# theEricMa/TriplaneTurbo

Hardware: AMD Instinct MI355X
Metric: rendered rays/sec (fwd+bwd) at 256x256 rays x 128 samples (higher is better)
Workload: dtype f32 (fp32-grade: exact 3-piece fp16 operand split, 6 x v_mfma_f32_32x32x16_f16 per k-step, fp32 accumulation)

## Files before the change

### triplaneturbo_amd/csrc/tt_backward_common.h

```cpp
#pragma once
#include "tt_device.h"
#include "tt_mfma16.h"
#include "tt_alpha.h"
#include "tt_launch.h"
#include <type_traits>

typedef int i32x4 __attribute__((ext_vector_type(4)));

#ifdef TT_TUNING
#define TT_PHASE(k)                                              \
    do {                                                         \
        __builtin_amdgcn_sched_barrier(0);                       \
        const unsigned long long t_now = __builtin_amdgcn_s_memtime(); \
        ph_acc[k] += t_now - ph_t;                               \
        ph_t = t_now;                                            \
        __builtin_amdgcn_sched_barrier(0);                       \
    } while (0)
#else
#define TT_PHASE(k) \
    do {            \
    } while (0)
#endif
#define XS 36

template <int N>
__device__ __forceinline__ void stage_rows(float* S, const float (&v)[N / 2], int j, int hi) {
#pragma unroll
    for (int r = 0; r < N / 2; ++r) S[LIDX(r, hi) * XS + j] = v[r];
}
template <int N, int OFF, int TOT>
__device__ __forceinline__ void stage_rows_sub(float* S, const float (&v)[TOT], int j, int hi) {
#pragma unroll
    for (int r = 0; r < N / 2; ++r) S[LIDX(r, hi) * XS + j] = v[OFF + r];
}
template <int N>
__device__ __forceinline__ void stage_rows_mask(float* S, const float (&v)[N / 2], int j, int hi) {
#pragma unroll
    for (int r = 0; r < N / 2; ++r) S[LIDX(r, hi) * XS + j] = v[r] > 0.f ? 1.f : 0.f;
}

template <int NX, int NY>
__device__ __forceinline__ void wgrad(f32x16 (&acc)[NX / 32][NY / 32], const float* Xs, const float* Ys, int i,
                                      int hi) {
#pragma unroll
    for (int t4 = 0; t4 < 4; ++t4) {
        f32x4 xa[NX / 32], yb[NY / 32];
#pragma unroll
        for (int m = 0; m < NX / 32; ++m)
            xa[m] = *reinterpret_cast<const f32x4*>(Xs + (32 * m + i) * XS + 16 * hi + 4 * t4);
#pragma unroll
        for (int n = 0; n < NY / 32; ++n)
            yb[n] = *reinterpret_cast<const f32x4*>(Ys + (32 * n + i) * XS + 16 * hi + 4 * t4);
#pragma unroll
        for (int k = 0; k < 4; ++k)
#pragma unroll
            for (int m = 0; m < NX / 32; ++m)
#pragma unroll
                for (int n = 0; n < NY / 32; ++n)
                    acc[m][n] = __builtin_amdgcn_mfma_f32_32x32x2f32(xa[m][k], yb[n][k], acc[m][n], 0, 0, 0);
    }
}

template <int NY>
__device__ __forceinline__ void wgrad_row(f32x16 (&acc)[NY / 32], const float* Xs, const float* Ys, int i, int hi) {
#pragma unroll
    for (int t4 = 0; t4 < 4; ++t4) {
        f32x4 yb[NY / 32];
        const f32x4 xa = *reinterpret_cast<const f32x4*>(Xs + i * XS + 16 * hi + 4 * t4);
#pragma unroll
        for (int n = 0; n < NY / 32; ++n)
            yb[n] = *reinterpret_cast<const f32x4*>(Ys + (32 * n + i) * XS + 16 * hi + 4 * t4);
#pragma unroll
        for (int k = 0; k < 4; ++k)
#pragma unroll
            for (int n = 0; n < NY / 32; ++n)
                acc[n] = __builtin_amdgcn_mfma_f32_32x32x2f32(xa[k], yb[n][k], acc[n], 0, 0, 0);
    }
}

typedef unsigned u32x4 __attribute__((ext_vector_type(4)));

__device__ __forceinline__ float wg16_scale(float bound) {
    int E = (int)(__builtin_bit_cast(unsigned, bound * 1.0001f) >> 23) & 0xff;
    E = E < 16 ? 16 : (E > 240 ? 240 : E);
    return __builtin_bit_cast(float, (unsigned)(268 - E) << 23);
}
__device__ __forceinline__ unsigned wg16_pack(float x) {
    unsigned out;
    float r;
    asm("v_cvt_pk_f16_f32 %0, %2, 0\n\t"
        "v_fma_mix_f32 %1, %2, 1.0, -%0 op_sel_hi:[0,0,1]\n\t"
        "v_cvt_pk_f16_f32 %0, %2, %1"
        : "=&v"(out), "=&v"(r)
        : "v"(x));
    return out;
}
template <int N>
__device__ __forceinline__ void stage_rows16(float* S, const float (&v)[N / 2], int j, int hi, float sc) {
    unsigned* U = reinterpret_cast<unsigned*>(S);
#pragma unroll
    for (int r = 0; r < N / 2; ++r) U[LIDX(r, hi) * XS + j] = wg16_pack(v[r] * sc);
}
template <int N, int OFF, int TOT>
__device__ __forceinline__ void stage_rows16_sub(float* S, const float (&v)[TOT], int j, int hi, float sc) {
    unsigned* U = reinterpret_cast<unsigned*>(S);
#pragma unroll
    for (int r = 0; r < N / 2; ++r) U[LIDX(r, hi) * XS + j] = wg16_pack(v[OFF + r] * sc);
}
template <int N, int PAIR, int NT>
__device__ __forceinline__ void stage_rows16_pre(float* S, const Split16<N, PAIR, NT>& v, int j, int hi) {
    unsigned* U = reinterpret_cast<unsigned*>(S);
#pragma unroll
    for (int t = 0; t < N / 4; ++t) {
        U[LIDX(pair_reg<PAIR>(t, 0), hi) * XS + j] = __builtin_amdgcn_perm(v.l[t], v.h[t], 0x05040100u);
        U[LIDX(pair_reg<PAIR>(t, 1), hi) * XS + j] = __builtin_amdgcn_perm(v.l[t], v.h[t], 0x07060302u);
    }
}
template <int N>
__device__ __forceinline__ void stage_rows16_mask(float* S, const unsigned (&mb)[N / 4], int j, int hi) {
    unsigned* U = reinterpret_cast<unsigned*>(S);
#pragma unroll
    for (int t = 0; t < N / 4; ++t) {
        U[LIDX(2 * t, hi) * XS + j] = __builtin_amdgcn_perm(0u, mb[t], 0x01000100u);
        U[LIDX(2 * t + 1, hi) * XS + j] = __builtin_amdgcn_perm(0u, mb[t], 0x03020302u);
    }
}
__device__ __forceinline__ h8_t wg16_frag(const float* S, int row, int t, int hi) {
    return __builtin_bit_cast(h8_t, *reinterpret_cast<const u32x4*>(S + row * XS + 8 * t + 4 * hi));
}
__device__ __forceinline__ h8_t wg16_swap(h8_t v) {
    u32x4 u = __builtin_bit_cast(u32x4, v);
#pragma unroll
    for (int d = 0; d < 4; ++d) u[d] = __builtin_amdgcn_alignbit(u[d], u[d], 16);
    return __builtin_bit_cast(h8_t, u);
}
template <int NX, int NY>
__device__ __forceinline__ void wgrad16(f32x16 (&acc)[NX / 32][NY / 32], const float* Xs, const float* Ys, int i,
                                        int hi) {
#pragma unroll
    for (int t = 0; t < 4; ++t) {
        h8_t xa[NX / 32], yb[NY / 32], ys[NY / 32];
#pragma unroll
        for (int m = 0; m < NX / 32; ++m) xa[m] = wg16_frag(Xs, 32 * m + i, t, hi);
#pragma unroll
        for (int n = 0; n < NY / 32; ++n) {
            yb[n] = wg16_frag(Ys, 32 * n + i, t, hi);
            ys[n] = wg16_swap(yb[n]);
        }
#pragma unroll
        for (int m = 0; m < NX / 32; ++m)
#pragma unroll
            for (int n = 0; n < NY / 32; ++n)
                acc[m][n] = __builtin_amdgcn_mfma_f32_32x32x16_f16(xa[m], yb[n], acc[m][n], 0, 0, 0);
#pragma unroll
        for (int m = 0; m < NX / 32; ++m)
#pragma unroll
            for (int n = 0; n < NY / 32; ++n)
                acc[m][n] = __builtin_amdgcn_mfma_f32_32x32x16_f16(xa[m], ys[n], acc[m][n], 0, 0, 0);
    }
}
template <int NX, int NY>
__device__ __forceinline__ void wgrad16_mask(f32x16 (&acc)[NX / 32][NY / 32], const float* Xs, const float* Ys, int i,
                                             int hi) {
#pragma unroll
    for (int t = 0; t < 4; ++t) {
        h8_t xa[NX / 32], yb[NY / 32];
#pragma unroll
        for (int m = 0; m < NX / 32; ++m) xa[m] = wg16_frag(Xs, 32 * m + i, t, hi);
#pragma unroll
        for (int n = 0; n < NY / 32; ++n) yb[n] = wg16_frag(Ys, 32 * n + i, t, hi);
#pragma unroll
        for (int m = 0; m < NX / 32; ++m)
#pragma unroll
            for (int n = 0; n < NY / 32; ++n)
                acc[m][n] = __builtin_amdgcn_mfma_f32_32x32x16_f16(xa[m], yb[n], acc[m][n], 0, 0, 0);
    }
}
template <int NY>
__device__ __forceinline__ void wgrad16_row(f32x16 (&acc)[NY / 32], const float* Xs, const float* Ys, int i, int hi) {
#pragma unroll
    for (int t = 0; t < 4; ++t) {
        const h8_t xa = wg16_frag(Xs, i, t, hi);
        h8_t yb[NY / 32], ys[NY / 32];
#pragma unroll
        for (int n = 0; n < NY / 32; ++n) {
            yb[n] = wg16_frag(Ys, 32 * n + i, t, hi);
            ys[n] = wg16_swap(yb[n]);
        }
#pragma unroll
        for (int n = 0; n < NY / 32; ++n) acc[n] = __builtin_amdgcn_mfma_f32_32x32x16_f16(xa, yb[n], acc[n], 0, 0, 0);
#pragma unroll
        for (int n = 0; n < NY / 32; ++n) acc[n] = __builtin_amdgcn_mfma_f32_32x32x16_f16(xa, ys[n], acc[n], 0, 0, 0);
    }
}

__device__ __forceinline__ float block_max(float v, unsigned* word) {
    __syncthreads();
    if (threadIdx.x == 0) *word = 0u;
    __syncthreads();
#pragma unroll
    for (int o = 32; o > 0; o >>= 1) v = fmaxf(v, __shfl_xor(v, o));
    if ((threadIdx.x & 63) == 0) atomicMax(word, __builtin_bit_cast(unsigned, v));
    __syncthreads();
    const float r = __builtin_bit_cast(float, *word);
    __syncthreads();
    return r;
}

template <class Addr>
__device__ __forceinline__ void flush_tile_reduced(float* R, int parity, const f32x16& acc, int wave, int lane,
                                                   float ux, float uy, Addr addr) {
    float* B = R + parity * 4096;
#pragma unroll
    for (int r = 0; r < 16; ++r) B[(wave * 16 + r) * 64 + lane] = (acc[r] * ux) * uy;
    __syncthreads();
#pragma unroll
    for (int q = 0; q < 4; ++q) {
        const int r = 4 * wave + q;
        const float v = (B[r * 64 + lane] + B[(16 + r) * 64 + lane]) + (B[(32 + r) * 64 + lane] + B[(48 + r) * 64 + lane]);
        atomicAdd(addr(r), v);
    }
}
template <int NX, int NY>
__device__ __forceinline__ void flush_wgrad_reduced(float* R, int& parity, const f32x16 (&acc)[NX / 32][NY / 32],
                                                    float* __restrict__ dst, int wave, int lane, float ux, float uy) {
    const int i = lane & 31, hi = lane >> 5;
#pragma unroll
    for (int m = 0; m < NX / 32; ++m)
#pragma unroll
        for (int n = 0; n < NY / 32; ++n) {
            flush_tile_reduced(R, parity, acc[m][n], wave, lane, ux, uy,
                               [&](int r) { return dst + (32 * m + LIDX(r, hi)) * NY + 32 * n + i; });
            parity ^= 1;
        }
}

template <int NX, int NY>
__device__ __forceinline__ void flush_d_reduced(float* R, int& parity, const f32x16 (&acc)[NX / 32][NY / 32],
                                                const float* __restrict__ W, const float* __restrict__ wo,
                                                float* __restrict__ dW, float* __restrict__ dwo, int wave, int lane,
                                                float uy) {
    const int i = lane & 31, hi = lane >> 5;
#pragma unroll
    for (int m = 0; m < NX / 32; ++m) {
        float part[4] = {0.f, 0.f, 0.f, 0.f};
#pragma unroll
        for (int n = 0; n < NY / 32; ++n) {
            float* B = R + parity * 4096;
#pragma unroll
            for (int r = 0; r < 16; ++r) B[(wave * 16 + r) * 64 + lane] = acc[m][n][r] * uy;
            __syncthreads();
#pragma unroll
            for (int q = 0; q < 4; ++q) {
                const int r = 4 * wave + q, at = (32 * m + LIDX(r, hi)) * NY + 32 * n + i;
                const float d = (B[r * 64 + lane] + B[(16 + r) * 64 + lane]) + (B[(32 + r) * 64 + lane] + B[(48 + r) * 64 + lane]);
                atomicAdd(dW + at, wo[32 * m + LIDX(r, hi)] * d);
                part[q] = fmaf(W[at], d, part[q]);
            }
            parity ^= 1;
        }
#pragma unroll
        for (int q = 0; q < 4; ++q) {
            float s = part[q];
#pragma unroll
            for (int o = 16; o > 0; o >>= 1) s += __shfl_xor(s, o);
            if (i == 0) atomicAdd(dwo + 32 * m + LIDX(4 * wave + q, hi), s);
        }
    }
}

#define ZERO16 \
    { 0.f, 0.f, 0.f, 0.f, 0.f, 0.f, 0.f, 0.f, 0.f, 0.f, 0.f, 0.f, 0.f, 0.f, 0.f, 0.f }

#define MS XS

#define M16_RS 40
#define M16_PLANE (65 * M16_RS)
#define SCATTER_M_FLOATS 2624
template <bool EXACT>
__device__ __forceinline__ void scatter_clear(float* M, int lane) {
    const f32x4 z = {0.f, 0.f, 0.f, 0.f};
    if (EXACT) {
#pragma unroll
        for (int g = 0; g < MS / 4; ++g) *reinterpret_cast<f32x4*>(M + lane * MS + 4 * g) = z;
    } else {
#pragma unroll
        for (int g = 0; g < SCATTER_M_FLOATS / 256; ++g) *reinterpret_cast<f32x4*>(M + (g * 64 + lane) * 4) = z;
        if (lane < (SCATTER_M_FLOATS % 256) / 4)
            *reinterpret_cast<f32x4*>(M + ((SCATTER_M_FLOATS / 256) * 64 + lane) * 4) = z;
    }
}

#define SCATTER_TAG_INTS 160
__device__ __forceinline__ float* sc2_factor_table(int* tags, int pl) { return reinterpret_cast<float*>(tags + 32) + 32 * pl; }

struct PlaneRefs {
    float c0, c1;
    int o0, o1;
    int h0, h1;
    float qs;
};
template <bool NORM>
__device__ __forceinline__ PlaneRefs plane_refs(const float (&coef)[4], const int (&aoff)[4], const int (&hs)[4],
                                                int hi) {
    PlaneRefs r;
    float cn = 1.f;
    r.qs = 1.f;
    if (NORM) {
        const float m = fmaxf(fmaxf(__builtin_fabsf(coef[0]), __builtin_fabsf(coef[1])),
                              fmaxf(__builtin_fabsf(coef[2]), __builtin_fabsf(coef[3])));
        int E = (int)(__builtin_bit_cast(unsigned, m) >> 23);
        E = E < 16 ? 16 : (E > 240 ? 240 : E);
        cn = __builtin_bit_cast(float, (unsigned)(268 - E) << 23);
        r.qs = __builtin_bit_cast(float, (unsigned)(E - 14) << 23);
    }
    r.c0 = (hi ? coef[2] : coef[0]) * cn;
    r.c1 = (hi ? coef[3] : coef[1]) * cn;
    r.o0 = hi ? aoff[2] : aoff[0];
    r.o1 = hi ? aoff[3] : aoff[1];
    r.h0 = hi ? hs[2] : hs[0];
    r.h1 = hi ? hs[3] : hs[1];
    return r;
}
__device__ __forceinline__ void scatter_init_tags(int* tags, int lane) {
    if (lane < 32) tags[lane] = -2;
}
// ... 518 lines not shown
```

### triplaneturbo_amd/csrc/tt_backward_tex.hip

```cpp
#include "tt_backward_common.h"

#define TEX_SCRATCH_FLOATS (128 * XS)
template <int PREC>
struct TexMap : LdsMap<PREC, LdsImage<64, 96>, LdsImage<64, 64>, LdsRows<3, 64>, LdsImage<96, 64, PREC != PREC_S3>,
                       LdsImage<64, 64, PREC != PREC_S3>> {
    static constexpr bool COPIES = PREC != PREC_S3;
    typedef typename TexMap::template at<0> V1;
    typedef typename TexMap::template at<1> V2;
    typedef typename TexMap::template at<2> V3;
    typedef typename TexMap::template at<3> V1T;
    typedef typename TexMap::template at<4> V2T;
};
__device__ __forceinline__ float uniform_f(float v) {
    return __builtin_bit_cast(float, __builtin_amdgcn_readfirstlane(__builtin_bit_cast(int, v)));
}

template <int PREC, bool WG16, bool STATS = false>
__global__ __launch_bounds__(256, 1) void k_decode_bwd_tex(BwdTexParams p) {
    constexpr bool EXACT = PREC == PREC_F32;
    typedef TexMap<PREC> F;
    constexpr int NT = PrecNT<PREC>::value, WF = F::FLOATS;
    __shared__ __attribute__((aligned(16))) float Lt[WF + 4 * (TEX_SCRATCH_FLOATS + SCATTER_TAG_INTS)];
    stage_weights<PREC>(Lt, typename F::V1{}, p.w.v1);
    stage_weights<PREC>(Lt, typename F::V2{}, p.w.v2);
    stage_weights<PREC>(Lt, typename F::V3{}, p.w.v3);
    if constexpr (F::COPIES) {
        stage_weights_t<PREC>(Lt, typename F::V1T{}, p.w.v1);
        stage_weights_t<PREC>(Lt, typename F::V2T{}, p.w.v2);
    }
    const tt_render_cfg& cfg = p.cfg;
    float sKB1 = 1.f, sE = 1.f, sK2B = 1.f, sK1 = 1.f;
    if (WG16) {
        const unsigned* bnd = reinterpret_cast<const unsigned*>(p.queue) + TT_SLOT_BOUNDS;
        const float Pm = __builtin_bit_cast(float, bnd[TT_BOUND_PLANES]), Gr = __builtin_bit_cast(float, bnd[TT_BOUND_UP0]),
                    Gf = __builtin_bit_cast(float, bnd[TT_BOUND_UP1]);
        unsigned* word = reinterpret_cast<unsigned*>(Lt + WF);
        const int t = threadIdx.x;
        const float CBmax = __builtin_fabsf(cfg.rgb_grad_shrink) * (1.002f * 0.25f) * Gr + Gf;
        float v1row = 0.f, k2b = 0.f, kb1 = 0.f;
        if (t < 64) {
            for (int c = 0; c < 96; ++c) v1row += __builtin_fabsf(p.w.v1[t * 96 + c]);
            for (int o = 0; o < 3; ++o) k2b += __builtin_fabsf(p.w.v3[o * 64 + t]);
            for (int r = 0; r < 64; ++r) {
                float c3 = 0.f;
                for (int o = 0; o < 3; ++o) c3 += __builtin_fabsf(p.w.v3[o * 64 + r]);
                kb1 += __builtin_fabsf(p.w.v2[r * 64 + t]) * c3;
            }
        }
        const float V1max = block_max(v1row, word), K2Bw = block_max(k2b, word), KB1w = block_max(kb1, word);
        sE = wg16_scale(Pm);
        sK1 = wg16_scale(V1max * Pm);
        sK2B = wg16_scale(K2Bw * CBmax);
        sKB1 = wg16_scale(KB1w * CBmax);
    }
    sE = uniform_f(sE), sK1 = uniform_f(sK1), sK2B = uniform_f(sK2B), sKB1 = uniform_f(sKB1);
    const float uE = uniform_f(1.f / sE), uK1 = uniform_f(1.f / sK1);
    const TileGeom& tg = p.geom;
    const int lane = threadIdx.x & 63, i = lane & 31, hi = lane >> 5,
              wave_in_blk = __builtin_amdgcn_readfirstlane((int)(threadIdx.x >> 6));
    float* Xs = Lt + WF + wave_in_blk * (TEX_SCRATCH_FLOATS + SCATTER_TAG_INTS);
    float* Ys = Xs + 32 * XS;
    int* tags = reinterpret_cast<int*>(Xs + 128 * XS);
    float* Cb = Xs + 32;
#define CB_AT(idx) Cb[((idx) >> 2) * XS + ((idx)&3)]
    scatter_init_tags(tags, lane);
    __syncthreads();
    const int S = cfg.n_samples;
    const int H = cfg.plane_h, W = cfg.plane_w;
    const size_t HW = (size_t)H * W;
    const size_t plane_stride = 6 * HW * TT_C;
    ItemQueue iq = item_queue(p.queue, tg.n_blocks, tg.n_chunks, tg.unit);
    const float shrink = cfg.rgb_grad_shrink;
    float* const grad_out =
        p.grad_packed + (size_t)(blockIdx.x % (unsigned)p.n_copies) * cfg.n_prompts * plane_stride;
    const unsigned grad_bytes =
        TT_DBG(cfg.flags, TT_DBG_NO_ATOMICS) ? 0u : (unsigned)(cfg.n_prompts * plane_stride * sizeof(float));

    const TileStats st = STATS ? tile_stats(cfg.stats) : TileStats{nullptr};
    f32x16 accV1a[2][2] = {{ZERO16, ZERO16}, {ZERO16, ZERO16}};
    f32x16 accV1b[2][1] = {{ZERO16}, {ZERO16}};
    f32x16 accV2[2][2] = {{ZERO16, ZERO16}, {ZERO16, ZERO16}};
    float accV3[2][3] = {{0.f, 0.f, 0.f}, {0.f, 0.f, 0.f}};
#ifdef TT_TUNING
    unsigned long long ph_acc[20] = {0, 0, 0, 0, 0, 0, 0, 0, 0, 0, 0, 0, 0, 0, 0, 0, 0, 0, 0, 0};
    unsigned long long scat_st[3] = {0, 0, 0};
    unsigned long long ph_t = __builtin_amdgcn_s_memtime();
#endif

#pragma nounroll
    for (;;) {
      long long b;
      int ck;
      TT_PHASE(17);
      if (!item_pop(iq, tg.order, tg.n_chunks, b, ck)) break;
      TT_PHASE(18);
        if (b >= tg.n_blocks) continue;
      bool ray_ok;
      const long long ray = tile_ray(tg, b, i, ray_ok);
      const float ray_okf = tt_opaque(ray_ok ? 1.f : 0.f);
      const int ks = i % tg.sb;
      const int view = (int)(ray / cfg.rays_per_view);
      const size_t pofs = (size_t)(view / cfg.views_per_prompt) * plane_stride;
      const int s_end = (ck + 1) * tg.chunk < S ? (ck + 1) * tg.chunk : S;
      TT_PHASE(19);
      struct StepIn {
          float wgt, f[3], gf[3], ts, te;
      };
      auto load_step = [&](int sb0) {
          StepIn r;
          const int si = sb0 + ks;
          const long long sidx = ray * S + (si < S ? si : S - 1);
          r.wgt = p.weights ? p.weights[sidx] : 0.f;
#pragma unroll
          for (int o = 0; o < 3; ++o) {
              r.f[o] = p.weights ? p.features[sidx * 3 + o] : 0.f;
              r.gf[o] = p.g_features ? p.g_features[sidx * 3 + o] : 0.f;
          }
          r.ts = p.rays_d ? p.t_starts[sidx] : 0.f;
          r.te = p.rays_d ? p.t_ends[sidx] : 0.f;
          return r;
      };
      StepIn in = load_step(ck * tg.chunk), in_next;
#pragma nounroll
      for (int sb0 = ck * tg.chunk; sb0 < s_end; sb0 += tg.sb, in = in_next) {
        in_next = load_step(sb0 + tg.sb);
        const int si = sb0 + ks;
        const bool valid = ray_ok && si < s_end;
        const float vf = ray_okf * (si < s_end ? 1.f : 0.f);
        long long rr = ray;
        asm volatile("" : "+v"(rr));
        const float ox = p.rays_o[rr * 3 + 0], oy = p.rays_o[rr * 3 + 1], oz = p.rays_o[rr * 3 + 2];
        const float dx = p.rays_d ? p.rays_d[rr * 3 + 0] : 0.f, dy = p.rays_d ? p.rays_d[rr * 3 + 1] : 0.f,
                    dz = p.rays_d ? p.rays_d[rr * 3 + 2] : 0.f;
        float grgb[3];
#pragma unroll
        for (int o = 0; o < 3; ++o) grgb[o] = p.g_rgb ? p.g_rgb[rr * 3 + o] : 0.f;
        float cb[3];
#pragma unroll
        for (int o = 0; o < 3; ++o) {
            const float s = sigmoid_(in.f[o]);
            const float c = shrink * in.wgt * grgb[o] * 1.002f * s * (1.f - s) + in.gf[o];
            cb[o] = c * vf;
        }
        tile_stat(st, TT_STAT_VISITED);
        TT_PHASE(0);
        if (!__any(!((__builtin_fabsf(cb[0]) + __builtin_fabsf(cb[1])) + __builtin_fabsf(cb[2]) <= cfg.skip_eps_tex)))
            continue;
#ifdef TT_TUNING
        {
            const unsigned long long live = __ballot(cb[0] != 0.f || cb[1] != 0.f || cb[2] != 0.f) & 0xffffffffull;
            const unsigned long long big = __ballot(fabsf(cb[0]) + fabsf(cb[1]) + fabsf(cb[2]) > 1e-12f) & 0xffffffffull;
            ph_acc[12] += 1;
            ph_acc[13] += __popcll(live);
            ph_acc[14] += __popcll(big);
        }
#endif
        float tm, px, py, pz;
        sample_position(ox, oy, oz, dx, dy, dz, in.ts, in.te, tm, px, py, pz);
        const float X = scale_coord(px, cfg.radius), Y = scale_coord(py, cfg.radius), Z = scale_coord(pz, cfg.radius);
        float e[48];
        unsigned pmask;
        const bool any =
            __any(gather_tex_c(p.packed, (unsigned)(pofs / TT_C), H, W, X, Y, Z, valid, lane, Xs, e, pmask,
                               tile_stat_ptr(st, TT_STAT_INBOUNDS)));
        TT_PHASE(1);
        if (!any) continue;
        const bool one = single_plane(pmask);
        const int pl1 = single_plane_index(pmask);
        tile_stat_executed(st, one);
        const bool region = cfg.flags >= 0;
        const bool region_w = WG16 ? true : region;
        const bool do_wgrad = region_w && !TT_DBG(cfg.flags, TT_DBG_NO_WGRAD);
        float k1[32], k2[32];
        if (WG16) {
            Split16<96, PAIR_SEQ, NT> es;
            split16_vec<96, PAIR_SEQ, NT>(e, sE, es);
            if (do_wgrad) stage_rows16_pre<96>(Ys, es, i, hi);
            TT_PHASE(2);
            if (one) {
                Split16<32, PAIR_SEQ, NT> e1s;
                live_split32(es, e1s);
                mv16_pre_ks(Lt, typename F::V1{}, e1s, 2 * pl1, uE, k1, i, hi);
            } else {
                mv16_pre(Lt, typename F::V1{}, es, uE, k1, i, hi);
            }
        } else {
            if (do_wgrad) stage_rows<96>(Ys, e, i, hi);
            TT_PHASE(2);
            if (one) {
                float e1[16];
                live_block16(e, e1);
                mvx_plane<PREC>(Lt, typename F::V1{}, e1, pl1, k1, i, hi);
            } else {
                mvx<PREC>(Lt, typename F::V1{}, e, k1, i, hi);
            }
        }
#pragma unroll
        for (int r = 0; r < 32; ++r) k1[r] = fmaxf(k1[r], 0.f);
        TT_PHASE(3);
        Split16<64, PAIR_SEQ, NT> k1s;
        if (WG16) {
            split16_vec<64, PAIR_SEQ, NT>(k1, sK1, k1s);
            mv16_pre(Lt, typename F::V2{}, k1s, uK1, k2, i, hi);
        } else {
            mvx<PREC>(Lt, typename F::V2{}, k1, k2, i, hi);
        }
#pragma unroll
        for (int r = 0; r < 32; ++r) k2[r] = fmaxf(k2[r], 0.f);
        TT_PHASE(4);
        if (hi == 0) {
            CB_AT(0 * 32 + i) = cb[0];
            CB_AT(1 * 32 + i) = cb[1];
            CB_AT(2 * 32 + i) = cb[2];
        }
#pragma unroll
        for (int h2 = 0; h2 < 2; ++h2) {
            if (h2 == 0)
                stage_rows_sub<32, 0, 32>(Xs, k2, i, hi);
            else
                stage_rows_sub<32, 16, 32>(Xs, k2, i, hi);
#pragma unroll
            for (int g = 0; g < 4; ++g) {
                const f32x4 kk = *reinterpret_cast<const f32x4*>(Xs + i * XS + 16 * hi + 4 * g);
#pragma unroll
                for (int o = 0; o < 3; ++o) {
                    const f32x4 cc = *reinterpret_cast<const f32x4*>(&CB_AT(o * 32 + 16 * hi + 4 * g));
                    accV3[h2][o] += (kk[0] * cc[0] + kk[1] * cc[1]) + (kk[2] * cc[2] + kk[3] * cc[3]);
                }
            }
        }
        TT_PHASE(5);
#pragma unroll
        for (int g = 0; g < 8; ++g) {
            f32x4 v0 = *reinterpret_cast<const f32x4*>(lds_at(Lt, typename F::V3{}) + 0 * 64 + 8 * g + 4 * hi);
            f32x4 v1 = *reinterpret_cast<const f32x4*>(lds_at(Lt, typename F::V3{}) + 1 * 64 + 8 * g + 4 * hi);
            f32x4 v2 = *reinterpret_cast<const f32x4*>(lds_at(Lt, typename F::V3{}) + 2 * 64 + 8 * g + 4 * hi);
#pragma unroll
            for (int e2 = 0; e2 < 4; ++e2) {
                const float t = fmaf(v0[e2], cb[0], fmaf(v1[e2], cb[1], v2[e2] * cb[2]));
                k2[4 * g + e2] = k2[4 * g + e2] > 0.f ? t : 0.f;
            }
        }
        float kb1[32];
        if constexpr (F::COPIES)
            mvtx_copy<PREC>(Lt, typename F::V2T{}, typename F::V2{}, k2, kb1, i, hi);
        else
            mvtx<PREC>(Lt, typename F::V2{}, k2, kb1, i, hi);
#pragma unroll
        for (int r = 0; r < 32; ++r) kb1[r] = k1[r] > 0.f ? kb1[r] : 0.f;
        TT_PHASE(6);
        if (do_wgrad) {
            __builtin_amdgcn_sched_barrier(0);
#pragma unroll
            for (int h2 = 0; h2 < 2; ++h2) {
                if (WG16) {
                    if (h2 == 0)
                        stage_rows16_sub<32, 0, 32>(Xs, kb1, i, hi, sKB1);
                    else
                        stage_rows16_sub<32, 16, 32>(Xs, kb1, i, hi, sKB1);
                    wgrad16_row<64>(accV1a[h2], Xs, Ys, i, hi);
                    wgrad16_row<32>(accV1b[h2], Xs, Ys + 64 * XS, i, hi);
                } else {
                    if (h2 == 0)
                        stage_rows_sub<32, 0, 32>(Xs, kb1, i, hi);
                    else
                        stage_rows_sub<32, 16, 32>(Xs, kb1, i, hi);
                    wgrad_row<64>(accV1a[h2], Xs, Ys, i, hi);
                    wgrad_row<32>(accV1b[h2], Xs, Ys + 64 * XS, i, hi);
                }
            }
            TT_PHASE(7);
            if (WG16) {
                stage_rows16<64>(Xs, k2, i, hi, sK2B);
                stage_rows16_pre<64>(Xs + 64 * XS, k1s, i, hi);
                wgrad16<64, 64>(accV2, Xs, Xs + 64 * XS, i, hi);
            } else {
                stage_rows<64>(Xs, k2, i, hi);
                stage_rows<64>(Xs + 64 * XS, k1, i, hi);
                wgrad<64, 64>(accV2, Xs, Xs + 64 * XS, i, hi);
            }
            TT_PHASE(8);
        }
        if (region && !TT_DBG(cfg.flags, TT_DBG_NO_SCATTER)) {
            float* M = Xs;
            float* Es = Xs + (EXACT ? 65 * XS : SCATTER_M_FLOATS);
            scatter_clear<EXACT>(M, lane);
            const int tex0 = (int)(pofs / TT_C);
            float eb[48], ueb = 1.f;
            if constexpr (EXACT)
                mvtx_copy<PREC>(Lt, typename F::V1T{}, typename F::V1{}, kb1, eb, i, hi);
            else if constexpr (F::COPIES)
                mvtx_copy<PREC, true, true>(Lt, typename F::V1T{}, typename F::V1{}, kb1, eb, i, hi, 1.f, &ueb);
            else
                mvtx<PREC, true, true>(Lt, typename F::V1{}, kb1, eb, i, hi, 1.f, &ueb);
            TT_PHASE(9);
            auto prep_plane = [&](int pl, PlaneRefs& refs, const float* ebp) {
                Corners c;
                corners_setup(PLANE_U(pl, X, Y, Z), PLANE_V(pl, X, Y, Z), H, W, valid, c);
                int aoff[4];
#pragma unroll
                for (int q4 = 0; q4 < 4; ++q4)
                    aoff[q4] = tex0 + (int)((3 + pl) * HW) + c.off[q4];
                refs = plane_refs<!EXACT>(c.w, aoff, c.hs, hi);
                if constexpr (EXACT) {
#pragma unroll
                    for (int r = 0; r < 16; ++r) Es[i * 33 + LIDX(r, hi)] = ebp[r] * refs.qs;
                } else {
                    sc2_factor_table(tags, pl)[i] = ueb * refs.qs;
                }
            };
            auto load_plane_b = [&](int pl, auto& B, const float* ebp) {
                if constexpr (EXACT)
                    sc2_load_b(Es, i, hi, B);
                else
                    sc2_regs_b(ebp, sc2_factor_table(tags, pl), hi, B);
            };
            auto stage_plane_q = [&](int pl, const float* ebp) {
                if constexpr (!EXACT) sc2_regs_stage_q(ebp, sc2_factor_table(tags, pl), Es, i, hi);
            };
#define EB_TILE(pl) (eb + 16 * (pl))
            if (one) {
                float eb1[16];
#pragma unroll
                for (int r = 0; r < 16; ++r) eb1[r] = pl1 == 0 ? eb[r] : (pl1 == 1 ? eb[16 + r] : eb[32 + r]);
                scatter_one_plane<EXACT>(
                    grad_out, grad_bytes, Es, M, tags, Es + 32 * 33, i, hi, pl1,
                    [&](int pl, PlaneRefs& refs) { prep_plane(pl, refs, eb1); },
                    [&](int pl, auto& B) { load_plane_b(pl, B, eb1); }, [&](int pl) { stage_plane_q(pl, eb1); }
#ifdef TT_TUNING
                    , scat_st
#endif
                );
                TT_PHASE(10);
                continue;
            }
            scatter_planes<EXACT>(
                grad_out, grad_bytes, Es, M, tags, Es + 32 * 33, i, hi,
                [&](int pl, PlaneRefs& refs) { prep_plane(pl, refs, EB_TILE(pl)); },
                [&](int pl, auto& B) { load_plane_b(pl, B, EB_TILE(pl)); }, [&](int pl) { stage_plane_q(pl, EB_TILE(pl)); }
#ifdef TT_TUNING
                , scat_st
#endif
            );
#undef EB_TILE
            TT_PHASE(10);
        }
      }
    }
#ifdef TT_TUNING
    TT_PHASE(11);
    ph_acc[15] = scat_st[0];
    ph_acc[16] = scat_st[1];
    if (p.phase_cycles && lane == 0)
        for (int k = 0; k < 20; ++k) atomicAdd(p.phase_cycles + k, ph_acc[k]);
#endif
    __syncthreads();
    int parity = 0;
    {
        const float u1 = 1.f / sKB1, u2 = 1.f / sE;
#pragma unroll
        for (int m = 0; m < 2; ++m) {
            float* const base = p.grads.v1 + (32 * m) * 96 + i;
            flush_tile_reduced(Lt, parity, accV1a[m][0], wave_in_blk, lane, u1, u2,
                               [&](int r) { return base + LIDX(r, hi) * 96; });
            parity ^= 1;
            flush_tile_reduced(Lt, parity, accV1a[m][1], wave_in_blk, lane, u1, u2,
                               [&](int r) { return base + LIDX(r, hi) * 96 + 32; });
            parity ^= 1;
            flush_tile_reduced(Lt, parity, accV1b[m][0], wave_in_blk, lane, u1, u2,
                               [&](int r) { return base + LIDX(r, hi) * 96 + 64; });
            parity ^= 1;
        }
    }
    flush_wgrad_reduced<64, 64>(Lt, parity, accV2, p.grads.v2, wave_in_blk, lane, 1.f / sK2B, 1.f / sK1);
#pragma unroll
    for (int h2 = 0; h2 < 2; ++h2)
#pragma unroll
        for (int o = 0; o < 3; ++o) atomicAdd(p.grads.v3 + o * 64 + 32 * h2 + i, accV3[h2][o]);
    tile_stats_flush(st);
}

static void launch_bwd_tex(const BwdTexParams& p0, long long blocks, hipStream_t s) {
    BwdTexParams p = p0;
#ifdef TT_TUNING
    p.phase_cycles = g_phase_cycles;
#else
    p.phase_cycles = nullptr;
#endif
    if (use_wg16(p.cfg)) {
        unsigned* bnd = reinterpret_cast<unsigned*>(p.queue) + TT_SLOT_BOUNDS;
        launch_planes_bound(p.packed, p.cfg, 3, bnd + TT_BOUND_PLANES, s);
        if (p.g_rgb)
            hipLaunchKernelGGL(k_absmax1, dim3(absmax_blocks(p.cfg.n_rays * 3)), dim3(256), 0, s, p.g_rgb,
                               (long long)p.cfg.n_rays * 3, bnd + TT_BOUND_UP0);
        if (p.g_features) {
            const long long n = p.cfg.n_rays * p.cfg.n_samples * 3;
            hipLaunchKernelGGL(k_absmax1, dim3(absmax_blocks(n)), dim3(256), 0, s, p.g_features, n, bnd + TT_BOUND_UP1);
        }
    }
    tt_dispatch_prec(tt_prec_of_r(p.cfg.flags), [&](auto P) {
        constexpr int PREC = decltype(P)::value;
        constexpr bool WG16 = PREC != PREC_F32;
        if (p.cfg.stats)
            hipLaunchKernelGGL((k_decode_bwd_tex<PREC, WG16, true>), dim3((unsigned)blocks), dim3(256), 0, s, p);
        else
            hipLaunchKernelGGL((k_decode_bwd_tex<PREC, WG16>), dim3((unsigned)blocks), dim3(256), 0, s, p);
    });
}

extern "C" int tt_render_bwd_tex(const float* packed, const tt_mlp_weights* w, const float* rays_o,
                                 const float* rays_d, const float* t_starts, const float* t_ends,
                                 const tt_render_cfg* cfg, const float* weights, const float* features,
                                 const float* g_rgb_fg, const float* g_features, float* grad_packed,
                                 const tt_mlp_grads* grads, void* stream) {
    int st = tt_validate_cfg(cfg);
    if (st != TT_OK) return st;
    if (!packed || !w || !rays_o || !rays_d || !t_starts || !t_ends || !weights || !features || !grad_packed ||
        !grads)
        return TT_ERR_BAD_ARG;
    if (!w->v1 || !w->v2 || !w->v3 || !grads->v1 || !grads->v2 || !grads->v3) return TT_ERR_BAD_ARG;
    if (grad_buffer_too_large(cfg)) return TT_ERR_UNSUPPORTED;
    int cus = tt_num_cus();
    if (cus <= 0) return TT_ERR_DEVICE;
    hipStream_t s = (hipStream_t)stream;
    BwdTexParams p;
    tt_fill_rays(p, packed, w, rays_o, rays_d, t_starts, t_ends, *cfg);
    p.cfg.flags |= debug_flags();
    p.weights = weights;
    p.features = features;
    p.g_rgb = g_rgb_fg;
    p.g_features = g_features;
    p.grad_packed = grad_packed;
    p.n_copies = cfg->grad_copies > 0 ? cfg->grad_copies : 1;
    p.grads = to_gptrs(grads);
    st = tt_plan_queue(cfg, 4LL * cus, s, &p.geom, &p.n_items, &p.queue, 12);
    if (st != TT_OK) return st;
    launch_bwd_tex(p, tt_persistent_blocks(p.n_items, cus, 4), s);
    return tt_check_launch();
}

extern "C" int tt_points_bwd_tex(const float* packed, const tt_mlp_weights* w, const float* points, int32_t n_batch,
                                 int64_t n_points, int32_t n_prompts, int32_t views_per_prompt, int32_t plane_h,
                                 int32_t plane_w, float radius, int32_t plane_base, int32_t flags,
                                 const float* g_features, float* grad_packed, const tt_mlp_grads* grads,
                                 void* stream) {
    tt_render_cfg cfg;
    int st = points_cfg(&cfg, n_batch, n_points, n_prompts, views_per_prompt, plane_h, plane_w, radius, 0.5f, 1,
                        flags);
    if (st != TT_OK) return st;
    if (grad_buffer_too_large(&cfg)) return TT_ERR_UNSUPPORTED;
    if (!packed || !w || !points || !g_features || !grad_packed || !grads) return TT_ERR_BAD_ARG;
    if (!w->v1 || !w->v2 || !w->v3 || !grads->v1 || !grads->v2 || !grads->v3) return TT_ERR_BAD_ARG;
    if (plane_base != 0 && plane_base != 3) return TT_ERR_BAD_ARG;
    int cus = tt_num_cus();
    if (cus <= 0) return TT_ERR_DEVICE;
    const ptrdiff_t shift = (ptrdiff_t)(plane_base - 3) * plane_h * plane_w * TT_C;
    hipStream_t s = (hipStream_t)stream;
    BwdTexParams p;
    tt_fill_rays(p, packed + shift, w, points, nullptr, nullptr, nullptr, cfg);
    p.weights = nullptr;
    p.features = nullptr;
    p.g_rgb = nullptr;
    p.g_features = g_features;
    p.grad_packed = grad_packed + shift;
    p.n_copies = 1;
    p.grads = to_gptrs(grads);
    st = tt_plan_queue(&cfg, 4LL * cus, s, &p.geom, &p.n_items, &p.queue);
    if (st != TT_OK) return st;
    launch_bwd_tex(p, tt_persistent_blocks(p.n_items, cus, 4), s);
    return tt_check_launch();
}
```

Baseline: 8.112 million.

## Reschedule per-step input prefetch and hoist ray loads in texture backward

Result: no change. 8.181 million, median of 6 (+0.9%).

```diff
diff --git a/triplaneturbo_amd/csrc/tt_backward_common.h b/triplaneturbo_amd/csrc/tt_backward_common.h
--- a/triplaneturbo_amd/csrc/tt_backward_common.h
+++ b/triplaneturbo_amd/csrc/tt_backward_common.h
@@ -22,6 +22,24 @@
     } while (0)
 #endif
 #define XS 36
+
+__device__ __forceinline__ int step_issue_point(int ks, float anchor) {
+    asm volatile("" : "+v"(ks) : "v"(anchor));
+    return ks;
+}
+template <typename T>
+__device__ __forceinline__ void step_land(T& v) {
+    asm volatile("" : "+v"(v));
+}
+__device__ __forceinline__ unsigned opt_mask(bool present) {
+    unsigned m = present ? ~0u : 0u;
+    asm volatile("" : "+v"(m));
+    return __builtin_amdgcn_readfirstlane(m);
+}
+__device__ __forceinline__ long long opt_index(unsigned mask, long long idx) { return idx & (long long)(int)mask; }
+__device__ __forceinline__ float opt_value(unsigned mask, float raw) {
+    return __builtin_bit_cast(float, __builtin_bit_cast(unsigned, raw) & mask);
+}
 
 template <int N>
 __device__ __forceinline__ void stage_rows(float* S, const float (&v)[N / 2], int j, int hi) {
diff --git a/triplaneturbo_amd/csrc/tt_backward_tex.hip b/triplaneturbo_amd/csrc/tt_backward_tex.hip
--- a/triplaneturbo_amd/csrc/tt_backward_tex.hip
+++ b/triplaneturbo_amd/csrc/tt_backward_tex.hip
@@ -76,6 +76,13 @@
     const unsigned grad_bytes =
         TT_DBG(cfg.flags, TT_DBG_NO_ATOMICS) ? 0u : (unsigned)(cfg.n_prompts * plane_stride * sizeof(float));
 
+    const unsigned m_w = opt_mask(p.weights != nullptr), m_gf = opt_mask(p.g_features != nullptr),
+                   m_t = opt_mask(p.rays_d != nullptr);
+    const float* const in_w = p.weights ? p.weights : p.rays_o;
+    const float* const in_f = p.weights ? p.features : p.rays_o;
+    const float* const in_gf = p.g_features ? p.g_features : p.rays_o;
+    const float* const in_ts = p.rays_d ? p.t_starts : p.rays_o;
+    const float* const in_te = p.rays_d ? p.t_ends : p.rays_o;
     const TileStats st = STATS ? tile_stats(cfg.stats) : TileStats{nullptr};
     f32x16 accV1a[2][2] = {{ZERO16, ZERO16}, {ZERO16, ZERO16}};
     f32x16 accV1b[2][1] = {{ZERO16}, {ZERO16}};
@@ -103,68 +110,108 @@
       const size_t pofs = (size_t)(view / cfg.views_per_prompt) * plane_stride;
       const int s_end = (ck + 1) * tg.chunk < S ? (ck + 1) * tg.chunk : S;
       TT_PHASE(19);
+      struct RayIn {
+          float o[3], d[3], g[3];
+      };
+      auto load_ray = [&](long long rr) {
+          RayIn r;
+#pragma unroll
+          for (int o = 0; o < 3; ++o) {
+              r.o[o] = p.rays_o[rr * 3 + o];
+              r.d[o] = p.rays_d ? p.rays_d[rr * 3 + o] : 0.f;
+              r.g[o] = p.g_rgb ? p.g_rgb[rr * 3 + o] : 0.f;
+          }
+          return r;
+      };
+      RayIn rc = load_ray(ray);
       struct StepIn {
           float wgt, f[3], gf[3], ts, te;
       };
-      auto load_step = [&](int sb0) {
+      auto load_step = [&](int sb0, int ks) {
           StepIn r;
           const int si = sb0 + ks;
           const long long sidx = ray * S + (si < S ? si : S - 1);
-          r.wgt = p.weights ? p.weights[sidx] : 0.f;
+          const long long sw = opt_index(m_w, sidx), sg = opt_index(m_gf, sidx), sq = opt_index(m_t, sidx);
+          r.wgt = in_w[sw];
 #pragma unroll
           for (int o = 0; o < 3; ++o) {
-              r.f[o] = p.weights ? p.features[sidx * 3 + o] : 0.f;
-              r.gf[o] = p.g_features ? p.g_features[sidx * 3 + o] : 0.f;
+              r.f[o] = in_f[sw * 3 + o];
+              r.gf[o] = in_gf[sg * 3 + o];
           }
-          r.ts = p.rays_d ? p.t_starts[sidx] : 0.f;
-          r.te = p.rays_d ? p.t_ends[sidx] : 0.f;
+          r.ts = in_ts[sq];
+          r.te = in_te[sq];
           return r;
       };
-      StepIn in = load_step(ck * tg.chunk), in_next;
+      auto use_step = [&](const StepIn& raw) {
+          StepIn r;
+          r.wgt = opt_value(m_w, raw.wgt), r.ts = opt_value(m_t, raw.ts), r.te = opt_value(m_t, raw.te);
+#pragma unroll
+          for (int o = 0; o < 3; ++o) r.f[o] = opt_value(m_w, raw.f[o]), r.gf[o] = opt_value(m_gf, raw.gf[o]);
+          return r;
+      };
+      auto land_step = [](StepIn& r) {
+          step_land(r.wgt), step_land(r.ts), step_land(r.te);
+#pragma unroll
+          for (int o = 0; o < 3; ++o) step_land(r.f[o]), step_land(r.gf[o]);
+      };
+      struct StepUp {
+          float cb[3], ts, te;
+      };
+      auto prep_step = [&](StepIn& raw, int sb0) {
+          land_step(raw);
+          const StepIn in = use_step(raw);
+          const float vf = ray_okf * (sb0 + ks < s_end ? 1.f : 0.f);
+          StepUp u;
+#pragma unroll
+          for (int o = 0; o < 3; ++o) {
+              const float s = sigmoid_(in.f[o]);
+              const float c = shrink * in.wgt * rc.g[o] * 1.002f * s * (1.f - s) + in.gf[o];
+              u.cb[o] = c * vf;
+          }
+          u.ts = in.ts, u.te = in.te;
+          return u;
+      };
+      StepIn in_next = load_step(ck * tg.chunk, ks);
+      StepUp up = prep_step(in_next, ck * tg.chunk), up_next;
 #pragma nounroll
-      for (int sb0 = ck * tg.chunk; sb0 < s_end; sb0 += tg.sb, in = in_next) {
-        in_next = load_step(sb0 + tg.sb);
+      for (int sb0 = ck * tg.chunk; sb0 < s_end; sb0 += tg.sb, up = up_next) {
         const int si = sb0 + ks;
         const bool valid = ray_ok && si < s_end;
-        const float vf = ray_okf * (si < s_end ? 1.f : 0.f);
-        long long rr = ray;
-        asm volatile("" : "+v"(rr));
-        const float ox = p.rays_o[rr * 3 + 0], oy = p.rays_o[rr * 3 + 1], oz = p.rays_o[rr * 3 + 2];
-        const float dx = p.rays_d ? p.rays_d[rr * 3 + 0] : 0.f, dy = p.rays_d ? p.rays_d[rr * 3 + 1] : 0.f,
-                    dz = p.rays_d ? p.rays_d[rr * 3 + 2] : 0.f;
-        float grgb[3];
-#pragma unroll
-        for (int o = 0; o < 3; ++o) grgb[o] = p.g_rgb ? p.g_rgb[rr * 3 + o] : 0.f;
-        float cb[3];
-#pragma unroll
-        for (int o = 0; o < 3; ++o) {
-            const float s = sigmoid_(in.f[o]);
-            const float c = shrink * in.wgt * grgb[o] * 1.002f * s * (1.f - s) + in.gf[o];
-            cb[o] = c * vf;
-        }
+        if constexpr (EXACT) {
+            long long rr = ray;
+            asm volatile("" : "+v"(rr));
+            rc = load_ray(rr);
+        }
+        const float cb[3] = {up.cb[0], up.cb[1], up.cb[2]};
         tile_stat(st, TT_STAT_VISITED);
         TT_PHASE(0);
-        if (!__any(!((__builtin_fabsf(cb[0]) + __builtin_fabsf(cb[1])) + __builtin_fabsf(cb[2]) <= cfg.skip_eps_tex)))
+        const bool upstream =
+            __any(!((__builtin_fabsf(cb[0]) + __builtin_fabsf(cb[1])) + __builtin_fabsf(cb[2]) <= cfg.skip_eps_tex));
+        float X, Y, Z, e[48];
+        unsigned pmask;
+        bool any = false;
+        if (upstream) {
+#ifdef TT_TUNING
+            {
+                const unsigned long long live = __ballot(cb[0] != 0.f || cb[1] != 0.f || cb[2] != 0.f) & 0xffffffffull;
+                const unsigned long long big = __ballot(fabsf(cb[0]) + fabsf(cb[1]) + fabsf(cb[2]) > 1e-12f) & 0xffffffffull;
+                ph_acc[12] += 1;
+                ph_acc[13] += __popcll(live);
+                ph_acc[14] += __popcll(big);
+            }
+#endif
+            float tm, px, py, pz;
+            sample_position(rc.o[0], rc.o[1], rc.o[2], rc.d[0], rc.d[1], rc.d[2], up.ts, up.te, tm, px, py, pz);
+            X = scale_coord(px, cfg.radius), Y = scale_coord(py, cfg.radius), Z = scale_coord(pz, cfg.radius);
+            any = __any(gather_tex_c(p.packed, (unsigned)(pofs / TT_C), H, W, X, Y, Z, valid, lane, Xs, e, pmask,
+                                     tile_stat_ptr(st, TT_STAT_INBOUNDS)));
+            TT_PHASE(1);
+        }
+        in_next = load_step(sb0 + tg.sb, step_issue_point(ks, any ? e[47] : cb[0]));
+        if (!any) {
+            up_next = prep_step(in_next, sb0 + tg.sb);
             continue;
-#ifdef TT_TUNING
-        {
-            const unsigned long long live = __ballot(cb[0] != 0.f || cb[1] != 0.f || cb[2] != 0.f) & 0xffffffffull;
-            const unsigned long long big = __ballot(fabsf(cb[0]) + fabsf(cb[1]) + fabsf(cb[2]) > 1e-12f) & 0xffffffffull;
-            ph_acc[12] += 1;
-            ph_acc[13] += __popcll(live);
-            ph_acc[14] += __popcll(big);
-        }
-#endif
-        float tm, px, py, pz;
-        sample_position(ox, oy, oz, dx, dy, dz, in.ts, in.te, tm, px, py, pz);
-        const float X = scale_coord(px, cfg.radius), Y = scale_coord(py, cfg.radius), Z = scale_coord(pz, cfg.radius);
-        float e[48];
-        unsigned pmask;
-        const bool any =
-            __any(gather_tex_c(p.packed, (unsigned)(pofs / TT_C), H, W, X, Y, Z, valid, lane, Xs, e, pmask,
-                               tile_stat_ptr(st, TT_STAT_INBOUNDS)));
-        TT_PHASE(1);
-        if (!any) continue;
+        }
         const bool one = single_plane(pmask);
         const int pl1 = single_plane_index(pmask);
         tile_stat_executed(st, one);
@@ -281,6 +328,7 @@
             }
             TT_PHASE(8);
         }
+        up_next = prep_step(in_next, sb0 + tg.sb);
         if (region && !TT_DBG(cfg.flags, TT_DBG_NO_SCATTER)) {
             float* M = Xs;
             float* Es = Xs + (EXACT ? 65 * XS : SCATTER_M_FLOATS);
```
